# guisongchen/vo_slam_test

Hardware: AMD Instinct MI355X
Metric: tracked frames/sec + local-BA LM-iters/sec (synthetic 640x480; value = tracked frames/sec: ORB extraction, frame post-processing, two guided searches with the culling / isInFrame steps between them and two pose-only solves per frame, one vo_tracker C call per batch) (higher is better)
Workload: dtype u8; 1 GPU; tracked frame: ORB extract (640x480, 8-level pyramid, 1000 kpts) + undistort/depth/grid + searchByProjection vs last frame + solvePoseOnlySE3 + cullingOutliersBeforeLocalMap + isInFrame (refined pose) + searchByProjection vs local map + solvePoseOnlySE3; frames, depth and map resident in HBM; parallelism=frames sharded x1, no collective, batches_in_flight=2

## Files before the change

include/vo_hip.h:

```cpp
#ifndef VO_HIP_H
#define VO_HIP_H

#include <stddef.h>
#include <stdint.h>

#ifdef __cplusplus
extern "C" {
#endif

typedef enum {
  VO_OK = 0,
  VO_ERR_INVALID = -1,
  VO_ERR_NO_DEVICE = -2,
  VO_ERR_HIP = -3,
  VO_ERR_CAPACITY = -4,
  VO_ERR_STOPPED = -5
} vo_status;

const char *vo_last_error(void);
int vo_device_count(void);
const char *vo_version(void);
size_t vo_release_thread_scratch(void);

typedef struct {
// ... 321 lines not shown
                                      const void *dev_depth, int depth_kind, size_t depth_frame_stride, int depth_pitch,
                                      const vo_tracker_params *params, int first_stage_only);
int vo_tracker_results(vo_tracker *t, double *poses6, double *Tcw12, int32_t *n_tracked, int32_t *n_inliers,
                       int32_t *n_matches_last, int32_t *n_matches_local, int32_t *status);
enum {
  VO_TRACKER_ASSIGNED_LAST = 0,
  VO_TRACKER_ASSIGNED_LOCAL = 1,
  VO_TRACKER_POSE_FIRST = 2,
  VO_TRACKER_INLIERS_FIRST = 3,
  VO_TRACKER_OBSERVED_INLIERS_FIRST = 4,
  VO_TRACKER_FEATURE_HAS_POINT = 5,
  VO_TRACKER_FEATURE_POINTS = 6,
  VO_TRACKER_LOCAL_FLAGS = 7, VO_TRACKER_LOCAL_U = 8, VO_TRACKER_LOCAL_V = 9, VO_TRACKER_LOCAL_UR = 10,
  VO_TRACKER_LOCAL_LEVEL = 11, VO_TRACKER_LOCAL_VIEWCOS = 12,
  VO_TRACKER_KEYPOINT_COUNTS = 13,
  VO_TRACKER_FEATURE_OUTLIER = 14
};
int vo_tracker_get(vo_tracker *t, int what, void *dst, size_t dst_bytes);
int vo_tracker_sync(vo_tracker *t);
#define VO_TRACKER_STAGES 6
int vo_tracker_set_timing(vo_tracker *t, int enabled);
int vo_tracker_get_timing(vo_tracker *t, double *ms , int *n_calls);

int vo_sim3_solve(int n_problems, const int32_t *offsets, const double *cam_match, const double *pix_curr,
                  const double *inv_sigma_curr, const double *cam_curr, const double *pix_match,
                  const double *inv_sigma_match, const double camera[4], int fix_scale, double *poses,
                  double *scales, uint8_t *outlier, int32_t *n_inliers, vo_lm_summary *summaries );

int vo_pose_graph_solve(int n_nodes, double *quats, double *trans, const double *scales, int fixed_node,
                        int n_edges, const int32_t *edge_i, const int32_t *edge_j, const double *q_meas,
                        const double *t_meas, const double *s_meas, int fix_scale, int max_iterations,
                        vo_lm_summary *summary);

int vo_sim3_reanchor_points(int n_points, const double *points_in, const int32_t *ref_node, int n_nodes,
                            const double *S_rw, const double *S_wr, double *points_out);

int vo_chol_solve(int n, double *A_rowmajor_lower, double *b);

int vo_chol_solve_split(int n, const double *A_rowmajor_lower, double *b, int c0_tiles, const int32_t *col_part, int n_ranks);

typedef struct vo_ba vo_ba;
int vo_ba_create(vo_ba **out, int n_cams, const double *poses, const uint8_t *cam_fixed, int n_points,
                 const double *points, int n_edges, const int32_t *edge_cam,
                 const int32_t *edge_point, const double *edge_obs, const double *edge_inv_sigma,
                 const double cam[5]);
void vo_ba_destroy(vo_ba *h);
int vo_ba_reset(vo_ba *h, int n_cams, const double *poses, const uint8_t *cam_fixed, int n_points, const double *points,
                int n_edges, const int32_t *edge_cam, const int32_t *edge_point, const double *edge_obs,
                const double *edge_inv_sigma, const double cam[5]);
int vo_ba_set_stream(vo_ba *h, void *hip_stream);
int vo_ba_set_shard(vo_ba *h, int shard, int n_shards);
enum { VO_BA_OPT_SEGMENTS = 1, VO_BA_OPT_COLLECTIVES_AT_ONE_RANK = 2, VO_BA_OPT_ORDER_PARTS = 3 };
int vo_ba_set_option(vo_ba *h, int option, int value);
enum { VO_OPT_BA_GRAPH = 1, VO_OPT_POSE_BLOCK = 2, VO_OPT_HAMMING_KERNEL = 3, VO_OPT_BA_PAIRS_KERNEL = 4 };
int vo_set_option(int option, int value);
typedef int (*vo_allreduce_fn)(void *user, double *dev_buf, size_t n_doubles, void *hip_stream);
int vo_ba_set_allreduce(vo_ba *h, vo_allreduce_fn fn, void *user);
int vo_ba_set_state(vo_ba *h, const double *poses, const double *points);
int vo_ba_get_state(vo_ba *h, double *poses, double *points);
int vo_ba_n_free_cams(const vo_ba *h);
int vo_ba_debug_order(vo_ba *h, int out[8]);

int vo_ba_local_ba(vo_ba *h, const volatile unsigned char *stop, uint8_t *edge_erase,
                   vo_lm_summary *summaries);
int vo_ba_local_ba_enqueue(vo_ba *h, const volatile unsigned char *stop);
int vo_ba_local_ba_finish(vo_ba *h, uint8_t *edge_erase, vo_lm_summary *summaries);
int vo_ba_solve(vo_ba *h, double huber_mono, double huber_stereo, int max_iterations,
                const uint8_t *edge_active, vo_lm_summary *summary);

int vo_ba_lm_begin(vo_ba *h, double huber_mono, double huber_stereo, int max_iterations,
                   const uint8_t *edge_active);
int vo_ba_linearize(vo_ba *h);
int vo_ba_step(vo_ba *h);
int vo_ba_update(vo_ba *h);
int vo_ba_lm_end(vo_ba *h, vo_lm_summary *summary);
int vo_ba_set_reduce_buffers(vo_ba *h, double *dev_system, double *dev_cost);
int vo_ba_reduced_system(vo_ba *h, double **dev_ptr, size_t *n_doubles);
int vo_ba_reduced_cost(vo_ba *h, double **dev_ptr, size_t *n_doubles);
int vo_ba_classify(vo_ba *h, int final_pass);
int vo_ba_lm_begin_inliers(vo_ba *h, double huber_mono, double huber_stereo, int max_iterations);
int vo_ba_get_edge_outliers(vo_ba *h, uint8_t *edge_erase);
int vo_ba_debug_schur(vo_ba *h, double huber_mono, double huber_stereo, double point_damping,
                      const uint8_t *edge_active, double *S, double *b, double *cost);

int vo_ba_debug_stamps(vo_ba *h, unsigned long long *out);

int vo_se3_exp(const double xi[6], double R_rowmajor[9], double t[3]);
int vo_se3_log(const double R_rowmajor[9], const double t[3], double xi[6]);

#ifdef __cplusplus
}
#endif
#endif
```

vo_slam_test_amd/_lib.py:

```python
from __future__ import annotations

import ctypes as C
import os
import pathlib

import numpy as np

PKG = pathlib.Path(__file__).resolve().parent
SO = PKG / "libvo_hip.so"

KP_DTYPE = np.dtype([("x", "<f4"), ("y", "<f4"), ("size", "<f4"), ("angle", "<f4"),
                     ("response", "<f4"), ("octave", "<i4"), ("class_id", "<i4")])


class VoError(RuntimeError):
    pass


class LmSummary(C.Structure):
    _fields_ = [("iterations", C.c_int32), ("accepted", C.c_int32), ("termination", C.c_int32),
                ("reserved", C.c_int32), ("initial_cost", C.c_double), ("final_cost", C.c_double),
                ("final_radius", C.c_double)]


# ... 794 lines not shown
        ninl = np.zeros(P, np.int32)
        sums = (LmSummary * (2 * P))()
        a_pm, a_pc, a_ic = cat("cam_match", 3), cat("pix_curr", 2), cat("isig_curr", 1)
        a_Pc, a_xm, a_im = cat("cam_curr", 3), cat("pix_match", 2), cat("isig_match", 1)
        check(lib().vo_sim3_solve(P, _p(offs), _p(a_pm), _p(a_pc), _p(a_ic), _p(a_Pc), _p(a_xm), _p(a_im), _p(cam),
                                  int(bool(fixScaleFlag)), _p(poses), _p(scales), _p(outl), _p(ninl),
                                  C.byref(sums) if summaries else None), "vo_sim3_solve")
        masks = [outl[offs[i]:offs[i + 1]].copy() for i in range(P)]
        if summaries:
            return poses, scales, masks, ninl, sums
        return poses, scales, masks, ninl


    @staticmethod
    def solvePoseGraphLoop(g, max_iterations=20):
        q = np.ascontiguousarray(g["quats"], np.float64).copy()
        t = np.ascontiguousarray(g["trans"], np.float64).copy()
        sc = np.ascontiguousarray(g["scales"], np.float64)
        ei, ej = np.ascontiguousarray(g["e_i"], np.int32), np.ascontiguousarray(g["e_j"], np.int32)
        qm, tm = np.ascontiguousarray(g["q_meas"], np.float64), np.ascontiguousarray(g["t_meas"], np.float64)
        sm = np.ascontiguousarray(g["s_meas"], np.float64)
        s = LmSummary()
        check(lib().vo_pose_graph_solve(len(q), _p(q), _p(t), _p(sc), int(g["fixed"]), len(ei), _p(ei), _p(ej), _p(qm),
                                        _p(tm), _p(sm), 1, int(max_iterations), C.byref(s)), "vo_pose_graph_solve")
        return q, t, s


def chol_solve(A, b):
    A = np.ascontiguousarray(A, np.float64).copy()
    x = np.ascontiguousarray(b, np.float64).copy()
    check(lib().vo_chol_solve(len(x), _p(A), _p(x)), "vo_chol_solve")
    return x, np.tril(A)


def chol_solve_split(A, b, c0_tiles, col_part, n_ranks):
    A = np.ascontiguousarray(A, np.float64)
    x = np.ascontiguousarray(b, np.float64).copy()
    cp = np.ascontiguousarray(col_part, np.int32)
    check(lib().vo_chol_solve_split(len(x), _p(A), _p(x), int(c0_tiles), _p(cp), int(n_ranks)), "vo_chol_solve_split")
    return x


def sim3_reanchor_points(points, ref, S_rw, S_wr):
    points = np.ascontiguousarray(points, np.float64)
    ref = np.ascontiguousarray(ref, np.int32)
    S_rw, S_wr = np.ascontiguousarray(S_rw, np.float64), np.ascontiguousarray(S_wr, np.float64)
    out = np.zeros_like(points)
    check(lib().vo_sim3_reanchor_points(len(points), _p(points), _p(ref), len(S_rw), _p(S_rw), _p(S_wr), _p(out)),
          "vo_sim3_reanchor_points")
    return out


def set_option(option, value):
    code = {"ba_graph": 1, "pose_block": 2, "hamming_kernel": 3, "ba_pairs_kernel": 4}.get(option, option)
    check(lib().vo_set_option(int(code), int(value)), "vo_set_option")


class BundleAdjuster:

    OPT_SEGMENTS, OPT_COLLECTIVES_AT_ONE_RANK, OPT_ORDER_PARTS = 1, 2, 3

    def __init__(self, prob, shard=0, n_shards=1, stream=None, options=None):
        self.prob = prob
        self.n_cams, self.n_pts, self.n_edges = len(prob["poses"]), len(prob["points"]), len(prob["e_cam"])
        self._h = C.c_void_p()
        a = {k: np.ascontiguousarray(v) for k, v in prob.items() if isinstance(v, np.ndarray)}
        check(lib().vo_ba_create(C.byref(self._h), self.n_cams, _p(a["poses"]), _p(a["fixed"]), self.n_pts,
                                 _p(a["points"]), self.n_edges, _p(a["e_cam"]), _p(a["e_pt"]), _p(a["e_obs"]),
                                 _p(a["e_inv_sigma"]), _p(a["cam"])), "vo_ba_create")
        if n_shards > 1:
            check(lib().vo_ba_set_shard(self._h, shard, n_shards), "vo_ba_set_shard")
        if stream is not None:
            check(lib().vo_ba_set_stream(self._h, C.c_void_p(stream)))
        for k, v in (options or {}).items():
            self.set_option(k, v)

    def reset(self, prob):
        self.prob = prob
        self.n_cams, self.n_pts, self.n_edges = len(prob["poses"]), len(prob["points"]), len(prob["e_cam"])
        a = {k: np.ascontiguousarray(v) for k, v in prob.items() if isinstance(v, np.ndarray)}
        check(lib().vo_ba_reset(self._h, self.n_cams, _p(a["poses"]), _p(a["fixed"]), self.n_pts, _p(a["points"]), self.n_edges,
                                _p(a["e_cam"]), _p(a["e_pt"]), _p(a["e_obs"]), _p(a["e_inv_sigma"]), _p(a["cam"])), "vo_ba_reset")

    def set_option(self, option, value):
        code = {"segments": 1, "collectives_at_one_rank": 2, "order_parts": 3}.get(option, option)
        check(lib().vo_ba_set_option(self._h, int(code), int(value)), "vo_ba_set_option")

    def close(self):
        if getattr(self, "_h", None) and self._h.value and _lib is not None:
            _lib.vo_ba_destroy(self._h)
            self._h = C.c_void_p()

    __del__ = close

    ALLREDUCE_FN = C.CFUNCTYPE(C.c_int, C.c_void_p, C.c_void_p, C.c_size_t, C.c_void_p)

    def set_allreduce(self, fn):
        self._ar = self.ALLREDUCE_FN(lambda user, buf, n, st: int(fn(buf, n, st) or 0))
        check(lib().vo_ba_set_allreduce(self._h, self._ar, None), "vo_ba_set_allreduce")

    def n_free_cams(self):
        return lib().vo_ba_n_free_cams(self._h)

    def state(self):
        poses = np.zeros((self.n_cams, 6))
        pts = np.zeros((self.n_pts, 3))
        check(lib().vo_ba_get_state(self._h, _p(poses), _p(pts)), "vo_ba_get_state")
# ... 257 lines not shown
```

vo_slam_test_amd/csrc/ba.hip:

```cpp
#include "ba_math.h"
#include "vo_common.h"

#include <algorithm>
#include <atomic>
#include <cmath>
#include <map>
#include <numeric>
#include <type_traits>
#include <vector>

namespace {

using namespace vo;
using namespace vo::ba;

template <int CTRL>
__device__ __forceinline__ double dpp_f64(double v) {
  const unsigned long long u = __double_as_longlong(v);
  const unsigned lo = (unsigned)__builtin_amdgcn_update_dpp(0, (int)(unsigned)u, CTRL, 0xf, 0xf, false);
  const unsigned hi = (unsigned)__builtin_amdgcn_update_dpp(0, (int)(unsigned)(u >> 32), CTRL, 0xf, 0xf, false);
  return __longlong_as_double(((unsigned long long)hi << 32) | lo);
}
__device__ __forceinline__ double readlane_f64(double v, int l) {
  const unsigned long long u = __double_as_longlong(v);
// ... 3626 lines not shown
  drop_graphs(h);
  if (h->own_stream) (void)hipStreamDestroy(h->stream);
  h->own_stream = false;
  h->stream = (hipStream_t)s;
  return VO_OK;
}

int vo_ba_set_shard(vo_ba *h, int shard, int n_shards) {
  if (!h || n_shards < 1 || shard < 0 || shard >= n_shards || h->built) {
    vo::set_error("vo_ba_set_shard: invalid argument or called after the first solve");
    return VO_ERR_INVALID;
  }
  h->shard = shard, h->n_shards = n_shards;
  return VO_OK;
}

int vo_ba_set_option(vo_ba *h, int option, int value) {
  if (!h || h->built) {
    vo::set_error("vo_ba_set_option: null handle or called after the first use of the handle");
    return VO_ERR_INVALID;
  }
  switch (option) {
    case VO_BA_OPT_SEGMENTS: h->opt_segments = value != 0; return VO_OK;
    case VO_BA_OPT_COLLECTIVES_AT_ONE_RANK: h->opt_collectives_1 = value != 0; return VO_OK;
    case VO_BA_OPT_ORDER_PARTS: h->opt_order_parts = value; return VO_OK;
    default: vo::set_error("vo_ba_set_option: unknown option %d", option); return VO_ERR_INVALID;
  }
}

int vo_set_option(int option, int value) {
  switch (option) {
    case VO_OPT_BA_GRAPH: g_opt_ba_graph.store(value != 0); return VO_OK;
    case VO_OPT_POSE_BLOCK:
      if (value != 0 && value != 64 && value != 128 && value != 256) {
        vo::set_error("vo_set_option(VO_OPT_POSE_BLOCK): 0 (automatic), 64, 128 or 256");
        return VO_ERR_INVALID;
      }
      g_opt_pose_block.store(value);
      return VO_OK;
    case VO_OPT_BA_PAIRS_KERNEL:
      if (value != 0 && value != 1) {
        vo::set_error("vo_set_option(VO_OPT_BA_PAIRS_KERNEL): 0 (blocks staged through LDS) or 1 (lane = couple, register loads)");
        return VO_ERR_INVALID;
      }
      g_opt_pairs_kernel.store(value);
      return VO_OK;
    case VO_OPT_HAMMING_KERNEL:
      if (value != 0 && value != 1) {
        vo::set_error("vo_set_option(VO_OPT_HAMMING_KERNEL): 0 (matrix cores) or 1 (VALU)");
        return VO_ERR_INVALID;
      }
      vo::set_hamming_kernel(value);
      return VO_OK;
    default: vo::set_error("vo_set_option: unknown option %d", option); return VO_ERR_INVALID;
  }
}

int vo_ba_n_free_cams(const vo_ba *h) { return h ? h->nf : 0; }

int vo_ba_debug_order(vo_ba *h, int out[8]) {
  if (!h || !out) return VO_ERR_INVALID;
  VO_CHECK(build_device(h));
  out[0] = h->order_parts, out[1] = h->order_cyclic, out[2] = h->order_sep, out[3] = h->order_depth, out[4] = h->order_tiles;
  out[5] = h->D.large ? h->D.ld / vo::kCholPanel : 0;
  out[6] = 0;
  out[7] = h->seg_mode ? h->seg_c0 : 0;
  vo::chol_plan_info(h->chol_plan, nullptr, nullptr, &out[6]);
  return VO_OK;
}

int vo_ba_set_state(vo_ba *h, const double *poses, const double *points) {
  if (!h) return VO_ERR_INVALID;
  VO_CHECK(build_device(h));
  h->state_cached = false;
  int cur;
  VO_CHECK(current_index(h, &cur));
  if (poses) VO_HIP_CHECK(hipMemcpy(h->D.Xc[cur], poses, (size_t)h->n_cams * 48, hipMemcpyHostToDevice));
  if (points && h->n_pts) VO_HIP_CHECK(hipMemcpy(h->D.Xp[cur], points, (size_t)h->n_pts * 24, hipMemcpyHostToDevice));
  return VO_OK;
}

static int merge_shards(vo_ba *h, int cur, uint8_t *erase_sorted ) {
  if (h->n_shards <= 1 || !h->allreduce || !h->built) return VO_OK;
  const size_t np3 = (size_t)h->n_pts * 3, n = np3 + (erase_sorted ? (size_t)h->n_edges : 0);
  if (n == 0) return VO_OK;
  std::vector<double> buf(n, 0.0);
  VO_HIP_CHECK(hipStreamSynchronize(h->stream));
  if (np3) VO_HIP_CHECK(hipMemcpy(buf.data(), h->D.Xp[cur], np3 * 8, hipMemcpyDeviceToHost));
  for (int j = 0; j < h->n_pts; j++)
    if (h->pt_owner[j] != h->shard) buf[3 * j] = buf[3 * j + 1] = buf[3 * j + 2] = 0.0;
  if (erase_sorted)
    for (int e = 0; e < h->n_edges; e++)
      buf[np3 + e] = (h->pt_owner[h->e_pt[e]] == h->shard && erase_sorted[e]) ? 1.0 : 0.0;
  VO_CHECK(h->b_merge.reserve(n * 8));
  VO_HIP_CHECK(hipMemcpyAsync(h->b_merge.p, buf.data(), n * 8, hipMemcpyHostToDevice, h->stream));
  VO_CHECK(shard_allreduce(h, h->b_merge.as<double>(), n));
  VO_HIP_CHECK(hipMemcpyAsync(buf.data(), h->b_merge.p, n * 8, hipMemcpyDeviceToHost, h->stream));
  if (np3) VO_HIP_CHECK(hipMemcpyAsync(h->D.Xp[cur], h->b_merge.p, np3 * 8, hipMemcpyDeviceToDevice, h->stream));
  VO_HIP_CHECK(hipStreamSynchronize(h->stream));
  if (erase_sorted)
    for (int e = 0; e < h->n_edges; e++) erase_sorted[e] = buf[np3 + e] != 0.0;
  return VO_OK;
}

int vo_ba_get_state(vo_ba *h, double *poses, double *points) {
  if (!h) return VO_ERR_INVALID;
// ... 291 lines not shown
```

vo_slam_test_amd/csrc/guided.hip:

```cpp
#include "vo_common.h"

#include <algorithm>
#include <cmath>
#include <vector>

namespace {

using namespace vo;

constexpr int kGridCols = 64, kGridRows = 48;
constexpr int kCells = kGridCols * kGridRows;
constexpr int TH_HIGH = 100, TH_LOW = 50;
constexpr int HISTO_LENGTH = 30;
constexpr int kMaxFeat = 16384;

enum GuidedMode {
  kModeFrame = 0,
  kModeLocalMap = 1,
  kModeKeyFrame = 2,
  kModeFuse = 3,
  kModeArea = 4,
  kModeSim3 = 5
};

struct FramesDev {
  int cap;
  float *x, *y, *angle, *uright, *depth;
  int *octave;
  uint8_t *desc;
  int *n;
  int *cell_start;
  unsigned short *cell_items;
  uint4 *srec;
  uint4 *sdesc;
  float xmin, ymin, gw, gh;
};

struct CamDev {
  float fx, fy, cx, cy, bf;
  double k[5];
  int distorted;
};

__global__ __launch_bounds__(256) void k_frame_post(FramesDev F, CamDev C, const vo_keypoint *kps, const uint8_t *desc,
                                                    const int *counts, int kp_capacity, const void *depth, int depth_kind,
                                                    long long depth_frame_stride, int depth_pitch, float inv_depth_scale,
                                                    int img_w, int img_h, int slot0, int *err) {
  const int f = blockIdx.y, i = blockIdx.x * 256 + threadIdx.x;
  const int n = min(counts[f], min(kp_capacity, F.cap));
  if (i == 0) {
    F.n[slot0 + f] = n;
    if (counts[f] > n) atomicOr(err, 2);
  }
  if (i >= n) return;
  const vo_keypoint kp = kps[(long long)f * kp_capacity + i];
// ... 124 lines not shown
  const int *nq;
  int nq_all, stride;
};

struct GuidedParams {
  int mode;
  float radius, bf, ratio, dist_threshold;
  int direction, check_rot, n_levels, max_dist;
  float sf[16];
  int retry_below;
};

constexpr float kNarrowRadius = 20.f;
constexpr int kSlot = 32;

struct GuidedOut {
  unsigned *pool;
  unsigned short *rank;
  unsigned *ovf;
  unsigned short *ovf_rank;
  uint2 *qrec;
  int *ovf_used;
  int ovf_stride;
  int *best_idx;
  int *assigned;
  const uint8_t *fmask;
  unsigned *pushes;
  int *n_matches;
  int *retry_nq;
  int *err;
};

__device__ __forceinline__ unsigned row_min_u32(unsigned x) {
  x = min(x, (unsigned)__builtin_amdgcn_update_dpp((int)x, (int)x, 0xB1, 0xf, 0xf, false));
  x = min(x, (unsigned)__builtin_amdgcn_update_dpp((int)x, (int)x, 0x4E, 0xf, 0xf, false));
  x = min(x, (unsigned)__builtin_amdgcn_update_dpp((int)x, (int)x, 0x141, 0xf, 0xf, false));
  x = min(x, (unsigned)__builtin_amdgcn_update_dpp((int)x, (int)x, 0x140, 0xf, 0xf, false));
  return x;
}
__device__ __forceinline__ unsigned wave_min_u32(unsigned x) {
  x = row_min_u32(x);
  return min(min((unsigned)__builtin_amdgcn_readlane((int)x, 0), (unsigned)__builtin_amdgcn_readlane((int)x, 16)),
             min((unsigned)__builtin_amdgcn_readlane((int)x, 32), (unsigned)__builtin_amdgcn_readlane((int)x, 48)));
}

template <int G>
__device__ __forceinline__ unsigned group_min_u32(unsigned x) {
  if (G == 16) return row_min_u32(x);
#pragma unroll
  for (int o = G / 2; o >= 1; o >>= 1) x = min(x, (unsigned)__shfl_xor((int)x, o, G));
  return x;
}

template <int G>
__global__ __launch_bounds__(256) void k_guided_cand(FramesDev F, Queries Q, GuidedParams P, GuidedOut O, int slot0) {
  constexpr int kMaxCol = 64, QPB = 256 / G;
  __shared__ int s_pre[QPB][kMaxCol], s_base[QPB][kMaxCol];
  const int lane = threadIdx.x & 63, l16 = threadIdx.x & (G - 1), grp = threadIdx.x / G, sub = lane / G;
  const int f = blockIdx.y, q = blockIdx.x * QPB + grp;
  const int nq = Q.nq ? Q.nq[f] : Q.nq_all;
  if (nq < 0) return;
  const bool live = q < nq;
  const long long qo = (long long)f * Q.stride + (live ? q : 0);
  const int s = slot0 + f;
  const bool claims = P.mode == kModeFrame || P.mode == kModeLocalMap || P.mode == kModeKeyFrame || P.mode == kModeSim3;
  const unsigned flags = live ? Q.flags[qo] : 0u;
  const bool valid = (flags & 1u) != 0;
  const float u = Q.u[qo], v = Q.v[qo];
  const int lv = min(max(Q.level[qo], 0), 15);
  const float aux = Q.aux ? Q.aux[qo] : 0.f;
  const float q_angle = (P.check_rot && Q.angle) ? Q.angle[qo] : 0.f;
  const uint4 *qd4 = reinterpret_cast<const uint4 *>(Q.desc + qo * 32);
  const uint4 qa = qd4[0], qb = qd4[1];
  float rs;
  int lmin, lmax;
  if (P.mode == kModeFrame) {
    rs = P.radius * P.sf[lv];
    if (P.direction == 1) lmin = lv, lmax = P.n_levels;
    else if (P.direction == 2) lmin = 0, lmax = lv;
    else lmin = lv - 1, lmax = lv + 1;
  } else if (P.mode == kModeLocalMap) {
    float r = (Q.viewcos ? Q.viewcos[qo] : 1.f) > 0.998 ? 2.5f : 4.0f;
    r *= P.radius;
    rs = r * P.sf[lv];
    lmin = lv - 1, lmax = lv;
  } else if (P.mode == kModeKeyFrame) {
    rs = P.radius * P.sf[lv];
    lmin = lv - 1, lmax = lv + 1;
  } else {
    rs = P.radius * P.sf[lv];
    lmin = -(1 << 30), lmax = 1 << 30;
  }
  const int x0 = max(0, (int)floorf((u - F.xmin - rs) * F.gw));
  const int x1 = min(kGridCols - 1, (int)floorf((u - F.xmin + rs) * F.gw));
  const int y0 = max(0, (int)floorf((v - F.ymin - rs) * F.gh));
  const int y1 = min(kGridRows - 1, (int)floorf((v - F.ymin + rs) * F.gh));
  const bool window = valid && !(x0 >= kGridCols || x1 < 0 || y0 >= kGridRows || y1 < 0 || x1 < x0 || y1 < y0);
  const int *start = F.cell_start + (long long)s * (kCells + 1);
  const long long fo = (long long)s * F.cap, mo = (long long)f * F.cap;
  const int ncol = window ? x1 - x0 + 1 : 0;
  int T = 0;
  for (int cb = 0; cb < kMaxCol; cb += G) {
    const int c = cb + l16;
    int cbeg = 0, ccnt = 0;
    if (c < ncol) {
      cbeg = start[(x0 + c) * kGridRows + y0];
      ccnt = start[(x0 + c) * kGridRows + y1 + 1] - cbeg;
    }
    int incl = ccnt;
#pragma unroll
    for (int o = 1; o < G; o <<= 1) {
      const int t = __shfl_up(incl, o, G);
      if (l16 >= o) incl += t;
    }
    s_pre[grp][c] = T + incl - ccnt;
    s_base[grp][c] = cbeg;
    T += __shfl(incl, G - 1, G);
    if (__builtin_amdgcn_ballot_w64(cb + G < ncol) == 0ull) break;
  }
  __builtin_amdgcn_fence(__ATOMIC_ACQ_REL, "wavefront");
  __builtin_amdgcn_wave_barrier();
  const float ur_q = P.mode == kModeFrame ? u - P.bf * aux : aux;
  const float pdf = HISTO_LENGTH / 360.0f;

  struct Item { bool inraw, pass; int idx, dist, oct, bin; };
  auto eval = [&](int t) {
    Item it{false, false, 0, 511, 0, 0};
    if (t >= T) return it;
    int lo = 0, hi = ncol - 1;
    while (lo < hi) {
      const int mid = (lo + hi + 1) >> 1;
      if (s_pre[grp][mid] <= t) lo = mid; else hi = mid - 1;
    }
    const long long pos = fo + s_base[grp][lo] + (t - s_pre[grp][lo]);
    const uint4 r = F.srec[pos];
    const uint4 da = F.sdesc[2 * pos], db = F.sdesc[2 * pos + 1];
    const float fx = __uint_as_float(r.x), fy = __uint_as_float(r.y), fur = __uint_as_float(r.z);
    const int oct = (int)(r.w & 0xffu), idx = (int)(r.w >> 8);
    it.idx = idx, it.oct = oct;
    if (oct < lmin || oct > lmax) return it;
    if (!(fabsf(fx - u) < rs && fabsf(fy - v) < rs)) return it;
    it.inraw = true;
    bool ok = true;
    if (P.mode == kModeFrame || P.mode == kModeLocalMap) {
      if (O.fmask && O.fmask[mo + idx]) ok = false;
// ... 42 lines not shown
    const int limit = P.mode == kModeFuse ? TH_LOW : P.max_dist;
    if (live && l16 == 0) O.best_idx[qo] = (best != 0xffffffffu && (int)(best >> 14) <= limit) ? (int)best_idx : -1;
    return;
  }

  unsigned *slot = O.pool + ((long long)f * Q.stride + (live ? q : 0)) * kSlot;
  unsigned short *rslot = O.rank ? O.rank + ((long long)f * Q.stride + (live ? q : 0)) * kSlot : nullptr;
  int written = 0, rawbase = 0;
  for (int base = 0; base < Tmax; base += G) {
    const Item it = eval(base + l16);
    const unsigned pm = (unsigned)(__builtin_amdgcn_ballot_w64(it.pass) >> (G * sub)) & kGroupMask;
    const unsigned rm = (unsigned)(__builtin_amdgcn_ballot_w64(it.inraw) >> (G * sub)) & kGroupMask;
    const unsigned below = (1u << l16) - 1u;
    if (it.pass) {
      const int p = written + __popc(pm & below);
      if (p < kSlot) {
        slot[p] = (unsigned)it.idx | ((unsigned)it.dist << 14) | ((unsigned)(it.oct & 15) << 23) | ((unsigned)it.bin << 27);
        if (rslot) rslot[p] = (unsigned short)min(rawbase + __popc(rm & below), 65535);
      }
    }
    written += __popc(pm);
    rawbase += __popc(rm);
  }
  int ovf_off = 0;
  if (__builtin_amdgcn_ballot_w64(written > kSlot) != 0ull) {
    if (written > kSlot) {
      if (l16 == 0) ovf_off = atomicAdd(&O.ovf_used[f], written - kSlot);
      ovf_off = __shfl(ovf_off, 0, G);
      if (ovf_off + written - kSlot > O.ovf_stride) {
        if (l16 == 0) atomicOr(O.err, 1);
        written = kSlot;
      }
    }
    unsigned *ov = O.ovf + (long long)f * O.ovf_stride + ovf_off - kSlot;
    unsigned short *orv = O.ovf_rank ? O.ovf_rank + (long long)f * O.ovf_stride + ovf_off - kSlot : nullptr;
    int w2 = 0, r2 = 0;
    for (int base = 0; base < Tmax; base += G) {
      const Item it = eval(base + l16);
      const unsigned pm = (unsigned)(__builtin_amdgcn_ballot_w64(it.pass) >> (G * sub)) & kGroupMask;
      const unsigned rm = (unsigned)(__builtin_amdgcn_ballot_w64(it.inraw) >> (G * sub)) & kGroupMask;
      const unsigned below = (1u << l16) - 1u;
      if (it.pass) {
        const int p = w2 + __popc(pm & below);
        if (p >= kSlot && p < written) {
          ov[p] = (unsigned)it.idx | ((unsigned)it.dist << 14) | ((unsigned)(it.oct & 15) << 23) | ((unsigned)it.bin << 27);
          if (orv) orv[p] = (unsigned short)min(r2 + __popc(rm & below), 65535);
        }
      }
      w2 += __popc(pm);
      r2 += __popc(rm);
    }
  }
  if (live && l16 == 0) O.qrec[qo] = make_uint2((unsigned)written | ((flags >> 1) & 1u) << 31, (unsigned)ovf_off);
}

__global__ __launch_bounds__(256) void k_features_in_area(FramesDev F, int slot, int nq, const float *qu, const float *qv,
                                                          const float *qr, const int *qlo, const int *qhi, int *out,
                                                          int max_out, int *count) {
  const int lane = threadIdx.x & 63, l16 = threadIdx.x & 15, sub = lane >> 4;
  const int q = blockIdx.x * 16 + (threadIdx.x >> 4);
  const bool live = q < nq;
  const int qq = live ? q : 0;
  const float u = qu[qq], v = qv[qq], rs = qr[qq];
  const int lmin = qlo ? qlo[qq] : -(1 << 30), lmax = qhi ? qhi[qq] : (1 << 30);
  const int x0 = max(0, (int)floorf((u - F.xmin - rs) * F.gw));
  const int x1 = min(kGridCols - 1, (int)floorf((u - F.xmin + rs) * F.gw));
  const int y0 = max(0, (int)floorf((v - F.ymin - rs) * F.gh));
  const int y1 = min(kGridRows - 1, (int)floorf((v - F.ymin + rs) * F.gh));
  const bool window = live && !(x0 >= kGridCols || x1 < 0 || y0 >= kGridRows || y1 < 0);
  const int *start = F.cell_start + (long long)slot * (kCells + 1);
  const long long fo = (long long)slot * F.cap;
  int written = 0;
  const int ncol = window ? x1 - x0 + 1 : 0;
  int ncmax = ncol;
#pragma unroll
  for (int o = 32; o >= 1; o >>= 1) ncmax = max(ncmax, __shfl_xor(ncmax, o));
  for (int c = 0; c < ncmax; c++) {
    int cbeg = 0, cend = 0;
    if (c < ncol && y1 >= y0) cbeg = start[(x0 + c) * kGridRows + y0], cend = start[(x0 + c) * kGridRows + y1 + 1];
    int len = cend - cbeg, lenmax = len;
#pragma unroll
    for (int o = 32; o >= 1; o >>= 1) lenmax = max(lenmax, __shfl_xor(lenmax, o));
    for (int base = 0; base < lenmax; base += 16) {
      const int t = base + l16;
      bool hit = false;
      int idx = 0;
      if (t < len) {
        const uint4 r = F.srec[fo + cbeg + t];
        const float fx = __uint_as_float(r.x), fy = __uint_as_float(r.y);
        const int oct = (int)(r.w & 0xffu);
        idx = (int)(r.w >> 8);
        hit = !(oct < lmin || oct > lmax) && fabsf(fx - u) < rs && fabsf(fy - v) < rs;
      }
      const unsigned m = (unsigned)(__builtin_amdgcn_ballot_w64(hit) >> (16 * sub)) & 0xffffu;
      if (hit) {
        const int p = written + __popc(m & ((1u << l16) - 1u));
        if (p < max_out) out[(long long)q * max_out + p] = idx;
      }
      written += __popc(m);
    }
  }
  if (live && l16 == 0) count[q] = written;
}

__device__ __forceinline__ void lds_handoff() {
  asm volatile("s_waitcnt lgkmcnt(0)" ::: "memory");
// ... 257 lines not shown
    else if (m3 < 0.1f * (float)m1) i3 = -1;
    __threadfence_block();
    for (int base = 0; base < npush; base += 64) {
      bool drop = false;
      if (base + lane < npush) {
        const unsigned p = pushes[base + lane];
        const int bin = (int)(p >> 16);
        if (bin != i1 && bin != i2 && bin != i3) {
          drop = true;
          asg[p & 0xffffu] = 0;
        }
      }
      cnt -= __popcll(__builtin_amdgcn_ballot_w64(drop));
    }
    lds_handoff();
  }
  const bool retry = O.retry_nq && cnt < P.retry_below;
  for (int i = lane; i < nf; i += 64) assigned[i] = retry ? -1 : (int)asg[i] - 1;
  if (lane == 0) {
    O.n_matches[f] = cnt, O.ovf_used[f] = 0;
    if (O.retry_nq) O.retry_nq[f] = retry ? nq : -1;
  }
}

__global__ __launch_bounds__(256) void k_guided_count(Queries Q, const int *best_idx, int *n_matches) {
  __shared__ int tot;
  const int f = blockIdx.x;
  const int nq = Q.nq ? Q.nq[f] : Q.nq_all;
  if (nq < 0) return;
  if (threadIdx.x == 0) tot = 0;
  __syncthreads();
  int c = 0;
  for (int q = threadIdx.x; q < nq; q += 256) c += best_idx[(long long)f * Q.stride + q] >= 0;
  if (c) atomicAdd(&tot, c);
  __syncthreads();
  if (threadIdx.x == 0) n_matches[f] = tot;
}

}

namespace vo {
void track_scatter_launch(int n_frames, int cap, int stride, const int *fn, int slot0, const int *assigned,
                          const double *qpoints, const uint8_t *qflags, double *fpoint, uint8_t *fhas, uint8_t *fobserved,
                          hipStream_t st);
void track_gather_launch(int n_frames, int cap, const int *fn, int slot0, const float *X, const float *Y, const float *UR,
                         const int *OCT, const double *fpoint, const uint8_t *fhas, const float *sf, double *pts, double *obs,
                         double *isg, int *ranges, int *index, hipStream_t st);
void track_scatter_gather_launch(int n_frames, int cap, int stride, const int *fn, int slot0, const int *assigned,
                                 const double *qpoints, const uint8_t *qflags, double *fpoint, uint8_t *fhas, uint8_t *fobserved,
                                 const float *X, const float *Y, const float *UR, const int *OCT, const float *sf, double *pts,
                                 double *obs, double *isg, int *ranges, int *index, hipStream_t st);
}

struct vo_frames {
  int max_frames = 0, cap = 0;
  FramesDev D{};
  CamDev cam{};
  float width = 640.f, height = 480.f;
  vo::DevBuf b_x, b_y, b_angle, b_ur, b_depth, b_oct, b_desc, b_n, b_cs, b_ci, b_srec, b_sdesc;
  vo::DevBuf b_pool, b_rank, b_ovf, b_ovfr, b_qrec, b_used, b_best, b_asg, b_push, b_nm, b_err, b_sf;
  size_t pool_stride = 0, replay_lds_attr = 0;
  float sf_host[16] = {0};
};

namespace {

int frames_alloc(vo_frames *h) {
  const size_t N = (size_t)h->max_frames * h->cap;
  VO_CHECK(h->b_x.reserve(N * 4));
  VO_CHECK(h->b_y.reserve(N * 4));
  VO_CHECK(h->b_angle.reserve(N * 4));
  VO_CHECK(h->b_ur.reserve(N * 4));
  VO_CHECK(h->b_depth.reserve(N * 4));
  VO_CHECK(h->b_oct.reserve(N * 4));
  VO_CHECK(h->b_desc.reserve(N * 32));
  VO_CHECK(h->b_n.reserve((size_t)h->max_frames * 4 + 64));
  VO_CHECK(h->b_cs.reserve((size_t)h->max_frames * (kCells + 1) * 4));
  VO_CHECK(h->b_ci.reserve(N * 2 + 64));
  VO_CHECK(h->b_srec.reserve(N * 16 + 64));
  VO_CHECK(h->b_sdesc.reserve(N * 32 + 64));
  FramesDev &D = h->D;
  D.cap = h->cap;
  D.x = h->b_x.as<float>(), D.y = h->b_y.as<float>(), D.angle = h->b_angle.as<float>();
  D.uright = h->b_ur.as<float>(), D.depth = h->b_depth.as<float>(), D.octave = h->b_oct.as<int>();
  D.desc = h->b_desc.as<uint8_t>(), D.n = h->b_n.as<int>(), D.cell_start = h->b_cs.as<int>();
  D.cell_items = h->b_ci.as<unsigned short>();
  D.srec = h->b_srec.as<uint4>(), D.sdesc = h->b_sdesc.as<uint4>();
  return VO_OK;
}

void frames_set_bounds(vo_frames *h, float xmin, float ymin, float xmax, float ymax) {
  h->D.xmin = xmin, h->D.ymin = ymin;
  h->D.gw = (float)kGridCols / (xmax - xmin);
  h->D.gh = (float)kGridRows / (ymax - ymin);
}

struct GuidedCall {
  int mode;
  float radius, bf, ratio, dist_threshold;
  int direction, check_rot, n_levels, max_dist;
  const float *scale_factors;
  int n_scale;
  int retry_below = 0;
  int *retry_nq = nullptr;
};

int guided_launch(vo_frames *h, int slot0, int n_frames, const Queries &Q, const GuidedCall &c, const uint8_t *fmask,
                  int *assigned, int *best_idx, int *n_matches, size_t pool_per_frame, hipStream_t st) {
  GuidedParams P{};
  P.mode = c.mode, P.radius = c.radius, P.bf = c.bf, P.ratio = c.ratio, P.dist_threshold = c.dist_threshold;
  P.direction = c.direction, P.check_rot = c.check_rot, P.n_levels = c.n_levels, P.max_dist = c.max_dist;
  for (int i = 0; i < 16; i++) P.sf[i] = i < c.n_scale ? c.scale_factors[i] : (c.n_scale > 0 ? c.scale_factors[c.n_scale - 1] : 1.f);
  const bool claims = c.mode == kModeFrame || c.mode == kModeLocalMap || c.mode == kModeKeyFrame || c.mode == kModeSim3;
  GuidedOut O{};
  O.best_idx = best_idx, O.assigned = assigned, O.fmask = fmask, O.n_matches = n_matches;
  P.retry_below = c.retry_below, O.retry_nq = c.retry_nq;
  if (!h->b_err.p) {
    VO_CHECK(h->b_err.reserve(64));
    VO_HIP_CHECK(hipMemsetAsync(h->b_err.p, 0, 64, st));
  }
  O.err = h->b_err.as<int>();
  if (claims) {
    const size_t slots = (size_t)n_frames * Q.stride * kSlot;
    VO_CHECK(h->b_pool.reserve(slots * 4 + 64));
    VO_CHECK(h->b_ovf.reserve((size_t)n_frames * pool_per_frame * 4 + 64));
    if (c.mode == kModeSim3) {
      VO_CHECK(h->b_rank.reserve(slots * 2 + 64));
      VO_CHECK(h->b_ovfr.reserve((size_t)n_frames * pool_per_frame * 2 + 64));
    }
    VO_CHECK(h->b_qrec.reserve((size_t)n_frames * Q.stride * 8 + 64));
    {
      void *before = h->b_used.p;
      VO_CHECK(h->b_used.reserve((size_t)h->max_frames * 4 + 64));
      if (h->b_used.p != before) VO_HIP_CHECK(hipMemsetAsync(h->b_used.p, 0, (size_t)h->max_frames * 4 + 64, st));
    }
    VO_CHECK(h->b_push.reserve((size_t)n_frames * Q.stride * 4 + 64));
    O.pool = h->b_pool.as<unsigned>(), O.ovf = h->b_ovf.as<unsigned>();
    O.rank = c.mode == kModeSim3 ? h->b_rank.as<unsigned short>() : nullptr;
    O.ovf_rank = c.mode == kModeSim3 ? h->b_ovfr.as<unsigned short>() : nullptr;
    O.qrec = h->b_qrec.as<uint2>(), O.ovf_used = h->b_used.as<int>(), O.pushes = h->b_push.as<unsigned>();
    O.ovf_stride = (int)pool_per_frame;
  }
  const int nq_max = Q.nq_all;
  if (nq_max > 0) {
    if (c.radius <= kNarrowRadius)
      hipLaunchKernelGGL(k_guided_cand<8>, dim3((nq_max + 31) / 32, n_frames), dim3(256), 0, st, h->D, Q, P, O, slot0);
    else
      hipLaunchKernelGGL(k_guided_cand<16>, dim3((nq_max + 15) / 16, n_frames), dim3(256), 0, st, h->D, Q, P, O, slot0);
  }
  if (claims) {
    const size_t capA = (size_t)((h->cap + 15) & ~15);
    const int batched = capA * 11 <= 160 * 1024 - 256 ? 1 : 0;
    const size_t lds = capA * 3 + (batched ? capA * 8 : 0);
    if (lds > 64 * 1024 && lds > h->replay_lds_attr) {
      VO_HIP_CHECK(hipFuncSetAttribute((const void *)k_guided_replay, hipFuncAttributeMaxDynamicSharedMemorySize, (int)lds));
      h->replay_lds_attr = lds;
    }
    hipLaunchKernelGGL(k_guided_replay, dim3(n_frames), dim3(64), lds, st, h->D, Q, P, O, slot0, batched);
  } else {
    hipLaunchKernelGGL(k_guided_count, dim3(n_frames), dim3(256), 0, st, Q, best_idx, n_matches);
  }
  VO_HIP_CHECK(hipGetLastError());
  return VO_OK;
}

}

extern "C" {

int vo_frames_create(vo_frames **out, int max_frames, int max_features) {
  if (!out || max_frames < 1 || max_features < 1 || max_features > kMaxFeat) {
    vo::set_error("vo_frames_create: 1 <= max_features <= %d", kMaxFeat);
    return VO_ERR_INVALID;
  }
  VO_CHECK(vo::ensure_device());
  vo_frames *h = new vo_frames();
  h->max_frames = max_frames, h->cap = max_features;
  const int rc = frames_alloc(h);
  if (rc != VO_OK) {
    vo_frames_destroy(h);
    return rc;
  }
  frames_set_bounds(h, 0.f, 0.f, 640.f, 480.f);
  const size_t lds = (size_t)((h->cap + 15) & ~15) + (size_t)h->cap * 2;
  if (lds > 48 * 1024)
    VO_HIP_CHECK(hipFuncSetAttribute((const void *)k_guided_replay, hipFuncAttributeMaxDynamicSharedMemorySize, (int)lds));
  *out = h;
  return VO_OK;
}

void vo_frames_destroy(vo_frames *h) {
  if (!h) return;
  for (vo::DevBuf *b : {&h->b_x, &h->b_y, &h->b_angle, &h->b_ur, &h->b_depth, &h->b_oct, &h->b_desc, &h->b_n, &h->b_cs,
                        &h->b_ci, &h->b_srec, &h->b_sdesc, &h->b_pool, &h->b_rank, &h->b_ovf, &h->b_ovfr, &h->b_qrec, &h->b_used, &h->b_best, &h->b_asg, &h->b_push,
                        &h->b_nm, &h->b_err, &h->b_sf})
    b->release();
  delete h;
}

int vo_frames_set_camera(vo_frames *h, const float intrinsics[5], const float dist_coef[5], float width, float height) {
  if (!h || !intrinsics || !(width > 0) || !(height > 0)) return VO_ERR_INVALID;
// ... 439 lines not shown
```

vo_slam_test_amd/csrc/vo_common.h:

```cpp
#pragma once
#include <hip/hip_runtime.h>
#include <utility>
#include <vector>

#include <cstdarg>
#include <cstdio>
#include <cstdlib>
#include <cstring>

#include "../../include/vo_hip.h"

namespace vo {

void set_error(const char *fmt, ...);
int ensure_device();

#define VO_HIP_CHECK(expr)                                                                 \
  do {                                                                                     \
    hipError_t _e = (expr);                                                                \
    if (_e != hipSuccess) {                                                                \
      vo::set_error("%s failed: %s (%s:%d)", #expr, hipGetErrorString(_e), __FILE__, __LINE__); \
      return VO_ERR_HIP;                                                                   \
    }                                                                                      \
  } while (0)
// ... 50 lines not shown
    const size_t want = n + n / 2 + 4096;
    VO_HIP_CHECK(hipHostMalloc(&p, want, hipHostMallocDefault));
    bytes = want;
    return VO_OK;
  }
  uint8_t *data() const { return reinterpret_cast<uint8_t *>(p); }
};

constexpr int kWave = 64;

hipStream_t thread_stream();
int copy_h2d(void *dst, const void *src, size_t bytes, hipStream_t st, const char *what);
int copy_d2h(void *dst, const void *src, size_t bytes, hipStream_t st, const char *what);
int stream_sync(hipStream_t st, const char *what);
int upload(DevBuf &b, const void *src, size_t bytes, hipStream_t st, const char *what);

constexpr int kCholPanel = 64;
size_t chol_workspace_bytes(int ld);
struct CholPlan;
CholPlan *chol_plan_create(int m, const unsigned long long *pattern);
void chol_plan_destroy(CholPlan *p);
void chol_plan_info(const CholPlan *p, int *n_tiles, int *depth, int *n_updates = nullptr);
void chol_symbolic(int m, const unsigned long long *pattern, unsigned long long *lmask, int *depth, int *n_tiles);
void chol_factor_solve(double *A, int ld, void *workspace, hipStream_t st, const CholPlan *plan = nullptr);
CholPlan *chol_plan_create_split(int m, const unsigned long long *pattern, int c0, unsigned long long own, int phase);
void chol_split_phase(double *A, int ld, void *workspace, hipStream_t st, const CholPlan *plan, int phase, int c0);
struct CholOrder {
  std::vector<int> slot_of;
  int parts = 1, cyclic = 0, sep = 0, depth = 0, tiles = 0;
  std::vector<unsigned long long> pattern;
  std::vector<int> part_of;
  int seg_slots = 0;
};
CholOrder chol_choose_order(int nf, int bs, const std::vector<std::pair<int, int>> &pairs, int m, int force_parts = -1);

struct RefKeyFrame {
  int n;
  const uint8_t *valid;
  const uint8_t *desc;
  const float *angle;
  const vo_bow_view *nodes;
};
int bow_search_resident(const vo_vocab *v, vo_frames *frames, int slot0, int B, const RefKeyFrame *kfs, float ratio, int check_rot,
                        int levelsup, int32_t *dev_assigned, int cap, int32_t *dev_n_matches, hipStream_t st);
struct FrameStoreView {
  int cap;
  const uint8_t *desc;
  const float *angle;
  const int *n;
};
FrameStoreView frame_store_view(const vo_frames *h);

void set_hamming_kernel(int v);

const int *orb_error_flag(const vo_orb *h);
const int *guided_error_flag(const vo_frames *h);

}
```

Measured before the change: 337,600 frames/s.

## Stage frame cell grid and feature records in LDS for guided candidate search

Adds a guided-search candidate kernel that loads the frame's cell-start table, the packed feature records and the match mask into LDS with async global-to-LDS loads. Each block then walks 256 queries against that copy instead of reading the grid from global memory per query. It is the default for wide-radius and local-map tracking searches when the LDS footprint fits in 48 KB. Lane grouping defaults to one lane per query and can be changed through new options. The cost is a per-block staging pass and lower occupancy from the LDS use. Searching each query with a single lane may also serialize long candidate lists.

```diff
diff --git a/include/vo_hip.h b/include/vo_hip.h
--- a/include/vo_hip.h
+++ b/include/vo_hip.h
@@ -397,7 +397,8 @@
 int vo_ba_set_shard(vo_ba *h, int shard, int n_shards);
 enum { VO_BA_OPT_SEGMENTS = 1, VO_BA_OPT_COLLECTIVES_AT_ONE_RANK = 2, VO_BA_OPT_ORDER_PARTS = 3 };
 int vo_ba_set_option(vo_ba *h, int option, int value);
-enum { VO_OPT_BA_GRAPH = 1, VO_OPT_POSE_BLOCK = 2, VO_OPT_HAMMING_KERNEL = 3, VO_OPT_BA_PAIRS_KERNEL = 4 };
+enum { VO_OPT_BA_GRAPH = 1, VO_OPT_POSE_BLOCK = 2, VO_OPT_HAMMING_KERNEL = 3, VO_OPT_BA_PAIRS_KERNEL = 4,
+       VO_OPT_GUIDED_KERNEL = 5, VO_OPT_GUIDED_LANES = 6 };
 int vo_set_option(int option, int value);
 typedef int (*vo_allreduce_fn)(void *user, double *dev_buf, size_t n_doubles, void *hip_stream);
 int vo_ba_set_allreduce(vo_ba *h, vo_allreduce_fn fn, void *user);
diff --git a/vo_slam_test_amd/_lib.py b/vo_slam_test_amd/_lib.py
--- a/vo_slam_test_amd/_lib.py
+++ b/vo_slam_test_amd/_lib.py
@@ -870,7 +870,7 @@
 
 
 def set_option(option, value):
-    code = {"ba_graph": 1, "pose_block": 2, "hamming_kernel": 3, "ba_pairs_kernel": 4}.get(option, option)
+    code = {"ba_graph": 1, "pose_block": 2, "hamming_kernel": 3, "ba_pairs_kernel": 4, "guided_kernel": 5, "guided_lanes": 6}.get(option, option)
     check(lib().vo_set_option(int(code), int(value)), "vo_set_option")
 
 
diff --git a/vo_slam_test_amd/csrc/ba.hip b/vo_slam_test_amd/csrc/ba.hip
--- a/vo_slam_test_amd/csrc/ba.hip
+++ b/vo_slam_test_amd/csrc/ba.hip
@@ -3702,6 +3702,20 @@
       }
       vo::set_hamming_kernel(value);
       return VO_OK;
+    case VO_OPT_GUIDED_KERNEL:
+      if (value != 0 && value != 1) {
+        vo::set_error("vo_set_option(VO_OPT_GUIDED_KERNEL): 0 (frame staged in LDS) or 1 (k_guided_cand)");
+        return VO_ERR_INVALID;
+      }
+      vo::set_guided_kernel(value);
+      return VO_OK;
+    case VO_OPT_GUIDED_LANES:
+      if (value != 0 && value != 1 && value != 2 && value != 4 && value != 8) {
+        vo::set_error("vo_set_option(VO_OPT_GUIDED_LANES): 0 (default), 1, 2, 4 or 8");
+        return VO_ERR_INVALID;
+      }
+      vo::set_guided_lanes(value);
+      return VO_OK;
     default: vo::set_error("vo_set_option: unknown option %d", option); return VO_ERR_INVALID;
   }
 }
diff --git a/vo_slam_test_amd/csrc/guided.hip b/vo_slam_test_amd/csrc/guided.hip
--- a/vo_slam_test_amd/csrc/guided.hip
+++ b/vo_slam_test_amd/csrc/guided.hip
@@ -1,6 +1,7 @@
 #include "vo_common.h"
 
 #include <algorithm>
+#include <atomic>
 #include <cmath>
 #include <vector>
 
@@ -231,6 +232,27 @@
   return x;
 }
 
+__device__ __forceinline__ void search_range(const Queries &Q, const GuidedParams &P, long long qo, int lv, float &rs,
+                                             int &lmin, int &lmax) {
+  if (P.mode == kModeFrame) {
+    rs = P.radius * P.sf[lv];
+    if (P.direction == 1) lmin = lv, lmax = P.n_levels;
+    else if (P.direction == 2) lmin = 0, lmax = lv;
+    else lmin = lv - 1, lmax = lv + 1;
+  } else if (P.mode == kModeLocalMap) {
+    float r = (Q.viewcos ? Q.viewcos[qo] : 1.f) > 0.998 ? 2.5f : 4.0f;
+    r *= P.radius;
+    rs = r * P.sf[lv];
+    lmin = lv - 1, lmax = lv;
+  } else if (P.mode == kModeKeyFrame) {
+    rs = P.radius * P.sf[lv];
+    lmin = lv - 1, lmax = lv + 1;
+  } else {
+    rs = P.radius * P.sf[lv];
+    lmin = -(1 << 30), lmax = 1 << 30;
+  }
+}
+
 template <int G>
 __global__ __launch_bounds__(256) void k_guided_cand(FramesDev F, Queries Q, GuidedParams P, GuidedOut O, int slot0) {
   constexpr int kMaxCol = 64, QPB = 256 / G;
@@ -253,23 +275,7 @@
   const uint4 qa = qd4[0], qb = qd4[1];
   float rs;
   int lmin, lmax;
-  if (P.mode == kModeFrame) {
-    rs = P.radius * P.sf[lv];
-    if (P.direction == 1) lmin = lv, lmax = P.n_levels;
-    else if (P.direction == 2) lmin = 0, lmax = lv;
-    else lmin = lv - 1, lmax = lv + 1;
-  } else if (P.mode == kModeLocalMap) {
-    float r = (Q.viewcos ? Q.viewcos[qo] : 1.f) > 0.998 ? 2.5f : 4.0f;
-    r *= P.radius;
-    rs = r * P.sf[lv];
-    lmin = lv - 1, lmax = lv;
-  } else if (P.mode == kModeKeyFrame) {
-    rs = P.radius * P.sf[lv];
-    lmin = lv - 1, lmax = lv + 1;
-  } else {
-    rs = P.radius * P.sf[lv];
-    lmin = -(1 << 30), lmax = 1 << 30;
-  }
+  search_range(Q, P, qo, lv, rs, lmin, lmax);
   const int x0 = max(0, (int)floorf((u - F.xmin - rs) * F.gw));
   const int x1 = min(kGridCols - 1, (int)floorf((u - F.xmin + rs) * F.gw));
   const int y0 = max(0, (int)floorf((v - F.ymin - rs) * F.gh));
@@ -418,6 +424,155 @@
     }
   }
   if (live && l16 == 0) O.qrec[qo] = make_uint2((unsigned)written | ((flags >> 1) & 1u) << 31, (unsigned)ovf_off);
+}
+
+typedef __attribute__((address_space(3))) uint8_t lds_u8;
+typedef const __attribute__((address_space(1))) uint8_t gmem_u8;
+constexpr int kLdsQueries = 256;
+constexpr int kCsBytes = ((kCells + 1) * 4 + 15) & ~15;
+constexpr float kLdsRadius = 2.f * kNarrowRadius;
+constexpr size_t kCandLdsBudget = 48 * 1024;
+__host__ __device__ constexpr size_t cand_lds_bytes(int cap) { return kCsBytes + ((cap + 15) & ~15) + (size_t)cap * 16; }
+
+template <int G>
+__global__ __launch_bounds__(256) void k_guided_cand_lds(FramesDev F, Queries Q, GuidedParams P, GuidedOut O, int slot0) {
+  extern __shared__ __attribute__((aligned(16))) uint8_t cl_lds[];
+  constexpr int QPB = 256 / G;
+  const int f = blockIdx.y, q0 = blockIdx.x * kLdsQueries;
+  const int nq = Q.nq ? Q.nq[f] : Q.nq_all;
+  if (q0 >= nq) return;
+  const int tid = threadIdx.x, lane = tid & 63, wave = __builtin_amdgcn_readfirstlane(tid >> 6);
+  const int s = slot0 + f;
+  const long long fo = (long long)s * F.cap, mo = (long long)f * F.cap;
+  const int capA = (F.cap + 15) & ~15;
+  const int *cs_g = F.cell_start + (long long)s * (kCells + 1);
+  const int total = min(cs_g[kCells], F.cap);
+  const int *cs = reinterpret_cast<const int *>(cl_lds);
+  uint8_t *fm = cl_lds + kCsBytes;
+  const uint4 *rec = reinterpret_cast<const uint4 *>(cl_lds + kCsBytes + capA);
+  for (int k = wave; k * 64 <= kCells; k += 4)
+    if (k * 64 + lane <= kCells)
+      __builtin_amdgcn_global_load_lds((gmem_u8 *)(cs_g + k * 64 + lane), (lds_u8 *)(cl_lds + 256 * k), 4, 0, 0);
+  for (int k = wave; k * 64 < total; k += 4)
+    if (k * 64 + lane < total)
+      __builtin_amdgcn_global_load_lds((gmem_u8 *)(F.srec + fo + k * 64 + lane),
+                                       (lds_u8 *)(cl_lds + kCsBytes + capA + 1024 * k), 16, 0, 0);
+  if (O.fmask) {
+    const int nf = min(F.n[s], F.cap);
+    for (int i = tid; i < nf; i += 256) fm[i] = O.fmask[mo + i];
+  }
+  asm volatile("s_waitcnt vmcnt(0)" ::: "memory");
+  __syncthreads();
+
+  const int l16 = tid & (G - 1), grp = tid / G, sub = lane / G;
+  constexpr unsigned kGroupMask = (1u << G) - 1u;
+  const unsigned below = (1u << l16) - 1u;
+  const float pdf = HISTO_LENGTH / 360.0f;
+  const int qend = min(q0 + kLdsQueries, nq);
+  for (int qb = q0; qb < qend; qb += QPB) {
+    const int q = qb + grp;
+    const bool live = q < qend;
+    if (__builtin_amdgcn_ballot_w64(live) == 0ull) break;
+    const long long qo = (long long)f * Q.stride + (live ? q : 0);
+    const unsigned flags = live ? Q.flags[qo] : 0u;
+    const bool valid = (flags & 1u) != 0;
+    const float u = Q.u[qo], v = Q.v[qo];
+    const int lv = min(max(Q.level[qo], 0), 15);
+    const float aux = Q.aux ? Q.aux[qo] : 0.f;
+    const float q_angle = (P.check_rot && Q.angle) ? Q.angle[qo] : 0.f;
+    const uint4 *qd4 = reinterpret_cast<const uint4 *>(Q.desc + qo * 32);
+    const uint4 qa = qd4[0], qb4 = qd4[1];
+    float rs;
+    int lmin, lmax;
+    search_range(Q, P, qo, lv, rs, lmin, lmax);
+    const int x0 = max(0, (int)floorf((u - F.xmin - rs) * F.gw));
+    const int x1 = min(kGridCols - 1, (int)floorf((u - F.xmin + rs) * F.gw));
+    const int y0 = max(0, (int)floorf((v - F.ymin - rs) * F.gh));
+    const int y1 = min(kGridRows - 1, (int)floorf((v - F.ymin + rs) * F.gh));
+    const bool window = valid && !(x0 >= kGridCols || x1 < 0 || y0 >= kGridRows || y1 < 0 || x1 < x0 || y1 < y0);
+    const int ncol = window ? x1 - x0 + 1 : 0;
+    int T = 0;
+    for (int c = 0; c < ncol; c++) T += cs[(x0 + c) * kGridRows + y1 + 1] - cs[(x0 + c) * kGridRows + y0];
+    const float ur_q = P.mode == kModeFrame ? u - P.bf * aux : aux;
+    int cc = 0, cum = 0, cb = 0, clen = 0;
+    auto rewind = [&]() {
+      cc = 0, cum = 0;
+      if (ncol) cb = cs[x0 * kGridRows + y0], clen = cs[x0 * kGridRows + y1 + 1] - cb;
+    };
+    auto seek = [&](int t) {
+      while (t >= cum + clen) {
+        cum += clen, cc++;
+        const int k = (x0 + cc) * kGridRows;
+        cb = cs[k + y0], clen = cs[k + y1 + 1] - cb;
+      }
+      return cb + (t - cum);
+    };
+    struct Item { bool pass; unsigned rec; };
+    auto eval = [&](int t) {
+      Item it{false, 0u};
+      if (t >= T) return it;
+      const int p = seek(t);
+      const uint4 r = rec[p];
+      const float fx = __uint_as_float(r.x), fy = __uint_as_float(r.y), fur = __uint_as_float(r.z);
+      const int oct = (int)(r.w & 0xffu), idx = (int)(r.w >> 8);
+      if (oct < lmin || oct > lmax) return it;
+      if (!(fabsf(fx - u) < rs && fabsf(fy - v) < rs)) return it;
+      if (O.fmask && fm[idx]) return it;
+      if (P.mode != kModeKeyFrame && fur > 0 && fabsf(ur_q - fur) > rs) return it;
+      it.pass = true;
+      const uint4 *d = F.sdesc + 2 * (fo + p);
+      const uint4 da = d[0], db = d[1];
+      int bin = 0;
+      if (P.check_rot && P.mode != kModeLocalMap) {
+        float rot = q_angle - F.angle[fo + idx];
+        if (rot < 0) rot += 360.0f;
+        bin = (int)rintf(rot * pdf);
+        if (bin == HISTO_LENGTH) bin = 0;
+        bin = min(max(bin, 0), 31);
+      }
+      const int dist = __popc(da.x ^ qa.x) + __popc(da.y ^ qa.y) + __popc(da.z ^ qa.z) + __popc(da.w ^ qa.w) +
+                       __popc(db.x ^ qb4.x) + __popc(db.y ^ qb4.y) + __popc(db.z ^ qb4.z) + __popc(db.w ^ qb4.w);
+      it.rec = (unsigned)idx | ((unsigned)dist << 14) | ((unsigned)(oct & 15) << 23) | ((unsigned)bin << 27);
+      return it;
+    };
+    const int Tmax = (int)(~wave_min_u32(~(unsigned)T));
+    unsigned *slot = O.pool + ((long long)f * Q.stride + (live ? q : 0)) * kSlot;
+    int written = 0;
+    rewind();
+    for (int base = 0; base < Tmax; base += G) {
+      const Item it = eval(base + l16);
+      const unsigned pm = (unsigned)(__builtin_amdgcn_ballot_w64(it.pass) >> (G * sub)) & kGroupMask;
+      if (it.pass) {
+        const int p = written + __popc(pm & below);
+        if (p < kSlot) slot[p] = it.rec;
+      }
+      written += __popc(pm);
+    }
+    int ovf_off = 0;
+    if (__builtin_amdgcn_ballot_w64(written > kSlot) != 0ull) {
+      if (written > kSlot) {
+        if (l16 == 0) ovf_off = atomicAdd(&O.ovf_used[f], written - kSlot);
+        if (G > 1) ovf_off = __shfl(ovf_off, 0, G);
+        if (ovf_off + written - kSlot > O.ovf_stride) {
+          if (l16 == 0) atomicOr(O.err, 1);
+          written = kSlot;
+        }
+      }
+      unsigned *ov = O.ovf + (long long)f * O.ovf_stride + ovf_off - kSlot;
+      int w2 = 0;
+      rewind();
+      for (int base = 0; base < Tmax; base += G) {
+        const Item it = eval(base + l16);
+        const unsigned pm = (unsigned)(__builtin_amdgcn_ballot_w64(it.pass) >> (G * sub)) & kGroupMask;
+        if (it.pass) {
+          const int p = w2 + __popc(pm & below);
+          if (p >= kSlot && p < written) ov[p] = it.rec;
+        }
+        w2 += __popc(pm);
+      }
+    }
+    if (live && l16 == 0) O.qrec[qo] = make_uint2((unsigned)written | ((flags >> 1) & 1u) << 31, (unsigned)ovf_off);
+  }
 }
 
 __global__ __launch_bounds__(256) void k_features_in_area(FramesDev F, int slot, int nq, const float *qu, const float *qv,
@@ -781,6 +936,12 @@
                                  double *obs, double *isg, int *ranges, int *index, hipStream_t st);
 }
 
+namespace vo {
+std::atomic<int> g_guided_kernel{0}, g_guided_lanes{0};
+void set_guided_kernel(int v) { g_guided_kernel.store(v); }
+void set_guided_lanes(int v) { g_guided_lanes.store(v); }
+}
+
 struct vo_frames {
   int max_frames = 0, cap = 0;
   FramesDev D{};
@@ -872,10 +1033,24 @@
   }
   const int nq_max = Q.nq_all;
   if (nq_max > 0) {
-    if (c.radius <= kNarrowRadius)
+    const size_t lds = cand_lds_bytes(h->cap);
+    const bool claims_tracking = c.mode == kModeFrame || c.mode == kModeLocalMap || c.mode == kModeKeyFrame;
+    const bool lds_form = vo::g_guided_kernel.load(std::memory_order_relaxed) == 0 && claims_tracking &&
+                          (c.mode == kModeLocalMap || c.radius > kNarrowRadius) && c.radius <= kLdsRadius &&
+                          lds <= kCandLdsBudget;
+    if (lds_form) {
+      const dim3 grid((nq_max + kLdsQueries - 1) / kLdsQueries, n_frames);
+      switch (vo::g_guided_lanes.load(std::memory_order_relaxed)) {
+        case 2: hipLaunchKernelGGL(k_guided_cand_lds<2>, grid, dim3(256), lds, st, h->D, Q, P, O, slot0); break;
+        case 4: hipLaunchKernelGGL(k_guided_cand_lds<4>, grid, dim3(256), lds, st, h->D, Q, P, O, slot0); break;
+        case 8: hipLaunchKernelGGL(k_guided_cand_lds<8>, grid, dim3(256), lds, st, h->D, Q, P, O, slot0); break;
+        default: hipLaunchKernelGGL(k_guided_cand_lds<1>, grid, dim3(256), lds, st, h->D, Q, P, O, slot0); break;
+      }
+    } else if (c.radius <= kNarrowRadius) {
       hipLaunchKernelGGL(k_guided_cand<8>, dim3((nq_max + 31) / 32, n_frames), dim3(256), 0, st, h->D, Q, P, O, slot0);
-    else
+    } else {
       hipLaunchKernelGGL(k_guided_cand<16>, dim3((nq_max + 15) / 16, n_frames), dim3(256), 0, st, h->D, Q, P, O, slot0);
+    }
   }
   if (claims) {
     const size_t capA = (size_t)((h->cap + 15) & ~15);
diff --git a/vo_slam_test_amd/csrc/vo_common.h b/vo_slam_test_amd/csrc/vo_common.h
--- a/vo_slam_test_amd/csrc/vo_common.h
+++ b/vo_slam_test_amd/csrc/vo_common.h
@@ -126,6 +126,8 @@
 FrameStoreView frame_store_view(const vo_frames *h);
 
 void set_hamming_kernel(int v);
+void set_guided_kernel(int v);
+void set_guided_lanes(int v);
 
 const int *orb_error_flag(const vo_orb *h);
 const int *guided_error_flag(const vo_frames *h);
```

New measurement: 342,600 frames/s, median of 6. 1.01x the previous value.
